# ParthaEth/GIF

Hardware: NVIDIA H100
Metric: G+D train step images/sec @256x256 bs32/GPU (higher is better)
Workload: dtype bf16x3 error-compensated tensor-core contraction (two-term bf16 operands, 3 MMAs per slice), f32 accumulate/storage

## Files before the change

gif_b200/_lib.py:

```python
import ctypes
import os

import torch

_HERE = os.path.dirname(os.path.abspath(__file__))
LIB_PATH = os.path.join(_HERE, "libgifb200.so")

_p = ctypes.c_void_p
_i = ctypes.c_int
_f = ctypes.c_float
_d = ctypes.c_double
_ll = ctypes.c_longlong
_sz = ctypes.c_size_t

SIGNATURES = {
    "gifb200_version": (_i, []),
    "gifb200_last_error": (ctypes.c_char_p, []),
    "gifb200_launch_count": (_ll, []),
    "gifb200_conv2d_workspace_bytes": (_sz, [_i] * 11),
    "gifb200_conv2d": (_i, [_p, _p, _p] + [_i] * 13 + [_p, _f, _f, _i, _p, _sz, _p]),
    "gifb200_conv2d_wgrad_workspace_bytes": (_sz, [_i] * 10),
    "gifb200_conv2d_wgrad_path": (_i, [_i] * 10),
    "gifb200_conv2d_wgrad": (_i, [_p, _p, _p] + [_i] * 12 + [_p, _sz, _p]),
    "gifb200_conv2d_ex_workspace_bytes": (_sz, [_i] * 13),
    "gifb200_conv2d_ex": (_i, [_p, _p, _p] + [_i] * 16 + [_p, _i, _p, _sz, _p]),
    "gifb200_pool2d": (_i, [_p, _p] + [_i] * 12 + [_p]),
    "gifb200_resize_bilinear": (_i, [_p, _p, _i, _i, _i, _ll, _ll, _ll, _ll, _i, _i, _i, _f, _f, _i, _p]),
    "gifb200_resize_bilinear_u8": (_i, [_p, _p, _i, _i, _i, _ll, _i, _i, _i, _f, _f, _i, _p]),
    "gifb200_split_bf16": (_i, [_p, _p, _p, _i, _i, _i, _p]),
    "gifb200_upfirdn2d": (_i, [_p, _p, _p] + [_i] * 14 + [_p]),
    "gifb200_bias_act": (_i, [_p, _p, _p, _p, _p, _i, _i, _i, _f, _f, _i, _p]),
    "gifb200_act_bwd": (_i, [_p, _p, _p, _ll, _f, _f, _i, _p]),
    "gifb200_rows_sum": (_i, [_p, _p, _i, _i, _i, _p]),
    "gifb200_chan_scale": (_i, [_p, _p, _p, _i, _i, _i, _i, _p]),
    "gifb200_tail_bwd": (_i, [_p] * 8 + [_i, _i, _i, _f, _f, _i, _p]),
# ... 86 lines not shown
```

gif_b200/csrc/conv_api.cu:

```cuda
#include "common.cuh"

namespace gifb200 {
int conv2d_simt(const float* x, const float* w, float* y, int B, int Hi, int Wi, int Ci, int Ho, int Wo, int Co, int k,
                int mode, int flip, int transposed, const ConvEpilogue& epi, cudaStream_t st);
int conv2d_wgrad_simt(const float* x, const float* gy, float* gw, int B, int Hi, int Wi, int Ci, int Ho, int Wo, int Co,
                      int k, int mode, int flip, int transposed, cudaStream_t st);
bool conv2d_tc_supported(int B, int Hi, int Wi, int Ci, int Ho, int Wo, int Co, int k, int mode);
size_t conv2d_tc_workspace_bytes(int B, int Hi, int Wi, int Ci, int Ho, int Wo, int Co, int k, int mode, int transposed);
int conv2d_tc(const float* x, const float* w, float* y, int B, int Hi, int Wi, int Ci, int Ho, int Wo, int Co, int k,
              int mode, int flip, int transposed, const ConvEpilogue& epi, void* ws, size_t ws_bytes, cudaStream_t st,
              bool x3, bool prestaged);
bool conv2d_wgrad_tc_supported(int B, int Hi, int Wi, int Ci, int Ho, int Wo, int Co, int k, int mode);
size_t conv2d_wgrad_tc_workspace_bytes(int B, int Hi, int Wi, int Ci, int Ho, int Wo, int Co, int k, int mode);
int conv2d_wgrad_tc(const float* x, const float* gy, float* gw, int B, int Hi, int Wi, int Ci, int Ho, int Wo, int Co,
                    int k, int mode, int flip, int transposed, void* ws, size_t ws_bytes, cudaStream_t st, bool x3);
}

using namespace gifb200;

extern "C" size_t gifb200_conv2d_workspace_bytes(int B, int Hi, int Wi, int Ci, int Ho, int Wo, int Co, int k, int mode,
                                                 int transposed, int impl) {
    impl &= 0xF;
    if (impl == 1) return 0;
    if (!conv2d_tc_supported(B, Hi, Wi, Ci, Ho, Wo, Co, k, mode)) return 0;
    return conv2d_tc_workspace_bytes(B, Hi, Wi, Ci, Ho, Wo, Co, k, mode, transposed);
}
// ... 4 lines not shown
                              gifb200_stream_t stream) {
    cudaStream_t st = static_cast<cudaStream_t>(stream);
    const ConvEpilogue epi{act, bias, slope, gain, round_tf32};
    const bool prestaged = (impl & GIFB200_CONV_PRESTAGED) != 0;
    impl &= 0xF;
    GIFB200_REQUIRE(impl >= 0 && impl <= 3, GIFB200_E_SHAPE,
                    "conv2d: impl must be 0 (auto), 1 (simt), 2 (wgmma tf32) or 3 (wgmma bf16x3 on split planes)");
    const bool tc_ok = conv2d_tc_supported(B, Hi, Wi, Ci, Ho, Wo, Co, k, mode);
    if (impl >= 2 && !tc_ok) return fail(GIFB200_E_SHAPE, "conv2d: shape not supported by the tensor-core path");
    if (impl != 1 && tc_ok)
        return conv2d_tc(x, w, y, B, Hi, Wi, Ci, Ho, Wo, Co, k, mode, flip, transposed, epi, workspace, workspace_bytes, st,
                         impl == 3, prestaged);
    return conv2d_simt(x, w, y, B, Hi, Wi, Ci, Ho, Wo, Co, k, mode, flip, transposed, epi, st);
}

extern "C" size_t gifb200_conv2d_wgrad_workspace_bytes(int B, int Hi, int Wi, int Ci, int Ho, int Wo, int Co, int k,
                                                       int mode, int impl) {
    if (impl == 1) return 0;
    return conv2d_wgrad_tc_workspace_bytes(B, Hi, Wi, Ci, Ho, Wo, Co, k, mode);
}

extern "C" int gifb200_conv2d_wgrad_path(int B, int Hi, int Wi, int Ci, int Ho, int Wo, int Co, int k, int mode, int impl) {
    if (impl == 1) return 1;
    if (conv2d_wgrad_tc_supported(B, Hi, Wi, Ci, Ho, Wo, Co, k, mode)) return impl == 3 ? 3 : 2;
    return impl == 0 ? 1 : 0;
}

extern "C" int gifb200_conv2d_wgrad(const float* x, const float* gy, float* gw, int B, int Hi, int Wi, int Ci, int Ho,
                                    int Wo, int Co, int k, int mode, int flip, int transposed, int impl, void* workspace,
                                    size_t workspace_bytes, gifb200_stream_t stream) {
// ... 10 lines not shown
```

gif_b200/csrc/conv_tc.cu:

```cuda
#include <cuda_bf16.h>

#include "tc_common.cuh"

namespace gifb200 {

namespace {

constexpr int kBlockK = 32;
constexpr int kMaxTaps = 9;
constexpr int kConsumerWarps = 8;

struct TcParams {
    int B, Hs, Ws;
    int wt, ht, nt;
    int tiles_x, tiles_y;
    int Ci, Co;
    int s2;
    int Ho, Wo;
    int oys, oxs;
    int nphase;
    int phase_oy0[4], phase_ox0[4], phase_ntaps[4];
    int tap_w[4][kMaxTaps];
    int tap_dy[4][kMaxTaps];
    int tap_dx[4][kMaxTaps];
    int tap_par[4][kMaxTaps];
    int in_sy;
    int ksplit;
    float* part;
    long long part_stride;
    ConvEpilogue epi;
};

constexpr int kProducerRegs = 40, kConsumerRegs = 232;
template <int BM, int BN>
struct TileCfg {
    static constexpr bool kLarge = BM * BN > 128 * 128;
    static constexpr int kRowBlocks = BM / 128;
    static constexpr int kAcc = kRowBlocks * BN / 2;
    static constexpr int kStages = kLarge ? 4 : 3;
    static constexpr int kThreads = kLarge ? 384 : 32 * kConsumerWarps + 32;
    static constexpr int kMinBlocks = kLarge ? 1 : 2;
    static constexpr int kATileBytes = BM * kBlockK * 4;
    static constexpr int kBTileBytes = BN * kBlockK * 4;
    static constexpr int kStageBytes = kATileBytes + kBTileBytes;
    static constexpr int kBarrierOffset = kStages * kStageBytes;
    static constexpr int kTotal = kBarrierOffset + 16 * kStages;
    static constexpr int kDynamic = kTotal + 1024;
    static_assert(kDynamic <= 227 * 1024, "shared memory ring too large");
};

__device__ __forceinline__ void decode_tile(int tile, int nblocks, int nphase, int rot_div, int& mt, int& nblk, int& phase) {
    const int inner = nblocks * nphase;
    mt = tile / inner;
    const int rem = tile - mt * inner;
    nblk = rem % nblocks;
    phase = nphase == 1 ? 0 : (rem / nblocks + mt / rot_div) % nphase;
}

template <int BM, int BN, bool X3>
__global__ void __launch_bounds__(TileCfg<BM, BN>::kThreads, TileCfg<BM, BN>::kMinBlocks)
    conv_tc_kernel(const __grid_constant__ CUtensorMap map_a, const __grid_constant__ CUtensorMap map_a2,
                   const __grid_constant__ CUtensorMap map_b, const __grid_constant__ CUtensorMap map_b2,
                   float* __restrict__ y, const TcParams p, const int mtiles, const int total_tiles) {
    using L = TileCfg<BM, BN>;
    constexpr int kStages = L::kStages;
    constexpr int kATileBytes = L::kATileBytes;
    extern __shared__ uint8_t smem_raw[];
    uint8_t* smem = reinterpret_cast<uint8_t*>((reinterpret_cast<uintptr_t>(smem_raw) + 1023) & ~static_cast<uintptr_t>(1023));
    uint64_t* full_bar = reinterpret_cast<uint64_t*>(smem + L::kBarrierOffset);
    uint64_t* empty_bar = full_bar + kStages;

    const int warp = threadIdx.x >> 5, lane = threadIdx.x & 31;
    const int nblocks = p.Co / BN;
    const int kchunks = p.Ci / kBlockK;
    const int rot_div = max(1, static_cast<int>(gridDim.x) / (nblocks * p.nphase));
    (void)mtiles;

    if (warp == kConsumerWarps && lane == 0) {
        asm volatile("prefetch.tensormap [%0];" ::"l"(&map_a) : "memory");
        asm volatile("prefetch.tensormap [%0];" ::"l"(&map_b) : "memory");
        if (X3) {
            asm volatile("prefetch.tensormap [%0];" ::"l"(&map_a2) : "memory");
            asm volatile("prefetch.tensormap [%0];" ::"l"(&map_b2) : "memory");
        }
        for (int s = 0; s < kStages; ++s) { mbar_init(&full_bar[s], 1); mbar_init(&empty_bar[s], 2); }
        asm volatile("fence.mbarrier_init.release.cluster;" ::: "memory");
        asm volatile("fence.proxy.async.shared::cta;" ::: "memory");
    }
    __syncthreads();

    if (warp >= kConsumerWarps) {
        if constexpr (L::kLarge) setmaxnreg_dec<kProducerRegs>();
        if (warp != kConsumerWarps) return;
        int stage = 0;
        uint32_t ph = 0;
        for (int tile = blockIdx.x; tile < total_tiles; tile += gridDim.x) {
            int mt, nblk, phase;
            const int ks = tile % p.ksplit;
            decode_tile(tile / p.ksplit, nblocks, p.nphase, rot_div, mt, nblk, phase);
            int m = mt;
            const int tx = m % p.tiles_x; m /= p.tiles_x;
            const int ty = m % p.tiles_y; m /= p.tiles_y;
            const int n0 = m * p.nt, y0 = ty * p.ht, x0 = tx * p.wt;
            const int iters = p.phase_ntaps[phase] * kchunks;
            const int it0 = iters * ks / p.ksplit, it1 = iters * (ks + 1) / p.ksplit;
            for (int it = it0; it < it1; ++it) {
                const int tap = it / kchunks, c0 = (it % kchunks) * kBlockK;
                uint8_t* a_dst = smem + stage * L::kStageBytes;
                uint8_t* b_dst = a_dst + kATileBytes;
                if (lane == 0) {
                    mbar_wait(&empty_bar[stage], ph ^ 1);
                    mbar_expect_tx(&full_bar[stage], L::kStageBytes);
                }
                __syncwarp();
                const int dy = p.tap_dy[phase][tap], dx = p.tap_dx[phase][tap];
                if (!p.s2) {
                    if (lane == 0) {
                        tma_load_4d(a_dst, &map_a, &full_bar[stage], c0, x0 + dx, y0 + dy, n0);
// ... 20 lines not shown
                }
                if (lane == 0) {
                    tma_load_3d(b_dst, &map_b, &full_bar[stage], c0, nblk * BN, p.tap_w[phase][tap]);
                    if (X3) tma_load_3d(b_dst + L::kBTileBytes / 2, &map_b2, &full_bar[stage], c0, nblk * BN, p.tap_w[phase][tap]);
                }
                if (++stage == kStages) { stage = 0; ph ^= 1; }
            }
        }
    } else {
        if constexpr (L::kLarge) setmaxnreg_inc<kConsumerRegs>();
        const int wg = warp >> 2;
        const int wq = warp & 3;
        constexpr int kRB = L::kRowBlocks;
        constexpr int kAcc = L::kAcc;
        float acc[kAcc];
        int w_in[2 * kRB], h_in[2 * kRB], n_in[2 * kRB];
#pragma unroll
        for (int rh = 0; rh < 2 * kRB; ++rh) {
            const int r = wg * (BM / 2) + (rh >> 1) * 64 + wq * 16 + (lane >> 2) + 8 * (rh & 1);
            w_in[rh] = r % p.wt; h_in[rh] = (r / p.wt) % p.ht; n_in[rh] = r / (p.wt * p.ht);
        }
        int stage = 0;
        uint32_t ph = 0;
        for (int tile = blockIdx.x; tile < total_tiles; tile += gridDim.x) {
            int mt, nblk, phase;
            const int ks = tile % p.ksplit;
            decode_tile(tile / p.ksplit, nblocks, p.nphase, rot_div, mt, nblk, phase);
            const int iters = p.phase_ntaps[phase] * kchunks;
            const int it0 = iters * ks / p.ksplit, it1 = iters * (ks + 1) / p.ksplit;
            int prev = -1;
            for (int it = it0; it < it1; ++it) {
                mbar_wait(&full_bar[stage], ph);
                const uint32_t a_addr = smem_u32(smem + stage * L::kStageBytes);
                wgmma_fence();
                fence_regs<kAcc>(acc);
                if (X3) {
                    const uint32_t a_wg = a_addr + wg * (BM / 2) * 64;
                    const uint64_t bh = make_kmajor_sw64_desc(a_addr + kATileBytes);
                    const uint64_t bl = make_kmajor_sw64_desc(a_addr + kATileBytes + L::kBTileBytes / 2);
#pragma unroll
                    for (int k = 0; k < kBlockK / 16; ++k) {
#pragma unroll
                        for (int rb = 0; rb < kRB; ++rb) {
                            const uint64_t ah = make_kmajor_sw64_desc(a_wg + rb * 64 * 64);
                            const uint64_t al = make_kmajor_sw64_desc(a_wg + rb * 64 * 64 + kATileBytes / 2);
                            float* d = acc + rb * (BN / 2);
                            wgmma_bf16<BN>(d, al + 2 * k, bh + 2 * k, (it != it0) || k != 0, Trans<0>());
                            wgmma_bf16<BN>(d, ah + 2 * k, bl + 2 * k, 1, Trans<0>());
                            wgmma_bf16<BN>(d, ah + 2 * k, bh + 2 * k, 1, Trans<0>());
                        }
                    }
                } else {
                    const uint64_t bdesc = make_kmajor_sw128_desc(a_addr + kATileBytes);
#pragma unroll
                    for (int k = 0; k < kBlockK / 8; ++k) {
#pragma unroll
                        for (int rb = 0; rb < kRB; ++rb) {
                            const uint64_t adesc = make_kmajor_sw128_desc(a_addr + (wg * (BM / 2) + rb * 64) * 128);
                            wgmma_tf32<BN>(acc + rb * (BN / 2), adesc + 2 * k, bdesc + 2 * k, (it != it0) || k != 0);
                        }
                    }
                }
                wgmma_commit();
                fence_regs<kAcc>(acc);
                wgmma_wait<1>();
                if (prev >= 0 && (threadIdx.x & 127) == 0) mbar_arrive(&empty_bar[prev]);
                prev = stage;
                if (++stage == kStages) { stage = 0; ph ^= 1; }
            }
            wgmma_wait<0>();
            fence_regs<kAcc>(acc);
            if (prev >= 0 && (threadIdx.x & 127) == 0) mbar_arrive(&empty_bar[prev]);
            int m = mt;
            const int tx = m % p.tiles_x; m /= p.tiles_x;
            const int ty = m % p.tiles_y; m /= p.tiles_y;
            float* base = p.ksplit > 1 ? p.part + ks * p.part_stride : y;
            const int c0 = nblk * BN + 2 * (lane & 3);
#pragma unroll
            for (int rh = 0; rh < 2 * kRB; ++rh) {
                const int h = rh & 1;
                const float* a = acc + (rh >> 1) * (BN / 2);
                const int n = m * p.nt + n_in[rh];
                const int Y = (ty * p.ht + h_in[rh]) * p.oys + p.phase_oy0[phase], X = (tx * p.wt + w_in[rh]) * p.oxs + p.phase_ox0[phase];
                if (n < p.B && Y < p.Ho && X < p.Wo) {
                    float* dst = base + ((static_cast<long long>(n) * p.Ho + Y) * p.Wo + X) * p.Co + c0;
#pragma unroll
                    for (int j = 0; j < BN / 8; ++j) {
                        float2 v = make_float2(a[4 * j + 2 * h], a[4 * j + 2 * h + 1]);
                        if (p.epi.act && p.ksplit == 1) {
                            v.x = apply_epilogue(p.epi, v.x, c0 + 8 * j);
                            v.y = apply_epilogue(p.epi, v.y, c0 + 8 * j + 1);
                        }
                        *reinterpret_cast<float2*>(dst + 8 * j) = v;
                    }
                }
            }
        }
    }
}

template <bool X3>
__global__ void __launch_bounds__(256) stage_weights_kernel(const float* __restrict__ w, float* __restrict__ out, int T,
                                                            int Co, int Ci, int flip, int transposed) {
    const long long total = static_cast<long long>(T) * Co * Ci;
    for (long long e = static_cast<long long>(blockIdx.x) * blockDim.x + threadIdx.x; e < total;
         e += static_cast<long long>(gridDim.x) * blockDim.x) {
        const int i = static_cast<int>(e % Ci);
        const int o = static_cast<int>((e / Ci) % Co);
        const int t = static_cast<int>(e / (static_cast<long long>(Ci) * Co));
        const int tt = flip ? T - 1 - t : t;
        const float v = transposed ? w[(static_cast<long long>(tt) * Ci + i) * Co + o]
                                   : w[(static_cast<long long>(tt) * Co + o) * Ci + i];
        if (X3) {
// ... 78 lines not shown
            a = fmaf(__bfloat162float(xv[i]) + __bfloat162float(xv[x_plane + i]),
                     __bfloat162float(wv[i]) + __bfloat162float(wv[w_plane + i]), a);
    } else {
        const float* xv = static_cast<const float*>(xpix_v) + b * x_batch_stride;
        const float* wv = static_cast<const float*>(w22_v) + static_cast<long long>(o) * Ci;
        for (int i = lane; i < Ci; i += 32) a = fmaf(xv[i], wv[i], a);
    }
    a = warp_sum(a);
    if (lane == 0) y[((static_cast<long long>(b) * Ho + (Ho - 1)) * Wo + (Wo - 1)) * Co + o] = apply_epilogue(epi, a, o);
}

void site_grid(int Hi, int Wi, int Ho, int Wo, int mode, int& Hs, int& Ws) {
    if (mode == 2) { Hs = Hi; Ws = Wi; } else { Hs = Ho; Ws = Wo; }
}

template <int BM, int BN, bool X3>
int launch(const CUtensorMap& ma, const CUtensorMap& ma2, const CUtensorMap& mb, const CUtensorMap& mb2, float* y,
           const TcParams& p, int mtiles, cudaStream_t st) {
    using L = TileCfg<BM, BN>;
    static bool attr_set = false;
    if (!attr_set) {
        cudaError_t e = cudaFuncSetAttribute(conv_tc_kernel<BM, BN, X3>, cudaFuncAttributeMaxDynamicSharedMemorySize, L::kDynamic);
        if (e != cudaSuccess) return fail(GIFB200_E_CUDA, "cudaFuncSetAttribute(conv_tc_kernel)", cudaGetErrorString(e));
        attr_set = true;
    }
    const long long total = static_cast<long long>(mtiles) * (p.Co / BN) * p.nphase * p.ksplit;
    if (total > 2147483647LL) return fail(GIFB200_E_SHAPE, "conv2d_tc: too many tiles");
    constexpr int kMaxGrid = L::kMinBlocks * kNumSMs;
    const int grid = total < kMaxGrid ? static_cast<int>(total) : kMaxGrid;
    conv_tc_kernel<BM, BN, X3><<<grid, L::kThreads, L::kDynamic, st>>>(ma, ma2, mb, mb2, y, p, mtiles, static_cast<int>(total));
    GIFB200_LAUNCH_CHECK("conv_tc_kernel");
    return GIFB200_OK;
}

template <bool X3>
int launch_tile(int bm, int bn, const CUtensorMap& ma, const CUtensorMap& ma2, const CUtensorMap& mb, const CUtensorMap& mb2,
                float* y, const TcParams& p, int mtiles, cudaStream_t st) {
    if (bm == 256) return launch<256, 128, X3>(ma, ma2, mb, mb2, y, p, mtiles, st);
    if (bn == 256) return launch<128, 256, X3>(ma, ma2, mb, mb2, y, p, mtiles, st);
    if (bn == 128) return launch<128, 128, X3>(ma, ma2, mb, mb2, y, p, mtiles, st);
    if (bn == 64) return launch<128, 64, X3>(ma, ma2, mb, mb2, y, p, mtiles, st);
    return launch<128, 32, X3>(ma, ma2, mb, mb2, y, p, mtiles, st);
}

int launch_any(int bm, int bn, bool x3, const CUtensorMap& ma, const CUtensorMap& ma2, const CUtensorMap& mb,
               const CUtensorMap& mb2, float* y, const TcParams& p, int mtiles, cudaStream_t st) {
    return x3 ? launch_tile<true>(bm, bn, ma, ma2, mb, mb2, y, p, mtiles, st)
              : launch_tile<false>(bm, bn, ma, ma2, mb, mb2, y, p, mtiles, st);
}

}

bool conv2d_tc_supported(int B, int Hi, int Wi, int Ci, int Ho, int Wo, int Co, int k, int mode) {
    if (B <= 0 || Ci % 32 != 0 || pick_block_n(Co) == 0) return false;
    if (!(k == 3 || (k == 1 && mode == 0))) return false;
    if (mode == 0 && !(Ho == Hi && Wo == Wi)) return false;
    if (mode == 1 && !(Hi == 2 * Ho + 1 && Wi == 2 * Wo + 1)) return false;
    if (mode == 2 && !(Ho == 2 * Hi + 1 && Wo == 2 * Wi + 1)) return false;
    int Hs, Ws;
    site_grid(Hi, Wi, Ho, Wo, mode, Hs, Ws);
    if (!pow2(Hs) || !pow2(Ws) || Ws < 4 || Hs < 4 || Ws > 4096 || Hs > 4096) return false;
    return true;
}

static size_t staged_weight_bytes(int Ci, int Co, int k) {
    return (static_cast<size_t>(k) * k * Co * Ci * sizeof(float) + 256 + 255) / 256 * 256;
}

static int ksplit_of(int B, int Hi, int Wi, int Ci, int Ho, int Wo, int Co, int k, int mode) {
    int Hs, Ws, wt, ht, nt;
    long long mtiles;
    site_grid(Hi, Wi, Ho, Wo, mode, Hs, Ws);
    tile_geometry(B, Hs, Ws, 128, wt, ht, nt, mtiles);
    const int bn = pick_block_n(Co);
    if (bn == 0) return 1;
    return pick_ksplit(mtiles * (Co / bn), k * k * (Ci / kBlockK), mode);
}

size_t conv2d_tc_workspace_bytes(int B, int Hi, int Wi, int Ci, int Ho, int Wo, int Co, int k, int mode, int) {
    size_t bytes = staged_weight_bytes(Ci, Co, k);
    if (conv2d_tc_supported(B, Hi, Wi, Ci, Ho, Wo, Co, k, mode)) {
        const int ks = ksplit_of(B, Hi, Wi, Ci, Ho, Wo, Co, k, mode);
        if (ks > 1) bytes += static_cast<size_t>(ks) * B * Ho * Wo * Co * sizeof(float) + 256;
    }
    return bytes;
}

int conv2d_tc(const float* x, const float* w, float* y, int B, int Hi, int Wi, int Ci, int Ho, int Wo, int Co, int k,
              int mode, int flip, int transposed, const ConvEpilogue& epi, void* ws, size_t ws_bytes, cudaStream_t st,
              bool x3, bool prestaged) {
    GIFB200_REQUIRE(conv2d_tc_supported(B, Hi, Wi, Ci, Ho, Wo, Co, k, mode), GIFB200_E_SHAPE, "conv2d_tc: unsupported shape");
// ... 23 lines not shown
    site_grid(Hi, Wi, Ho, Wo, mode, p.Hs, p.Ws);
    p.ksplit = ksplit_of(B, Hi, Wi, Ci, Ho, Wo, Co, k, mode);
    int bm, bn;
    pick_tile(B, p.Hs, p.Ws, Co, mode == 2 ? 4 : 1, p.ksplit, bm, bn);
    long long mtiles;
    tile_geometry(B, p.Hs, p.Ws, bm, p.wt, p.ht, p.nt, mtiles);
    p.tiles_x = p.Ws / p.wt; p.tiles_y = p.Hs / p.ht;
    GIFB200_REQUIRE(mtiles <= 2147483647LL, GIFB200_E_SHAPE, "conv2d_tc: too many tiles");
    if (p.ksplit > 1) {
        p.part_stride = static_cast<long long>(B) * Ho * Wo * Co;
        p.part = reinterpret_cast<float*>((reinterpret_cast<uintptr_t>(reinterpret_cast<char*>(wst) + staged_weight_bytes(Ci, Co, k) - 256) + 255) &
                                          ~static_cast<uintptr_t>(255));
    }
    p.s2 = mode == 1;
    p.in_sy = mode == 1 ? 2 : 1;
    const int pad = k / 2;
    if (mode == 0) {
        p.nphase = 1; p.oys = p.oxs = 1; p.phase_ntaps[0] = T;
        for (int t = 0; t < T; ++t) { p.tap_w[0][t] = t; p.tap_dy[0][t] = t / k - pad; p.tap_dx[0][t] = t % k - pad; }
    } else if (mode == 1) {
        p.nphase = 1; p.oys = p.oxs = 1; p.phase_ntaps[0] = T;
        for (int t = 0; t < T; ++t) {
            const int kh = t / k, kw = t % k;
            p.tap_w[0][t] = t; p.tap_dy[0][t] = kh; p.tap_dx[0][t] = kw >> 1; p.tap_par[0][t] = kw & 1;
        }
    } else {
        p.nphase = 4; p.oys = p.oxs = 2;
        for (int ph = 0; ph < 4; ++ph) {
            const int py = ph >> 1, px = ph & 1;
            p.phase_oy0[ph] = py; p.phase_ox0[ph] = px;
            int n = 0;
            for (int kh = py; kh < 3; kh += 2)
                for (int kw = px; kw < 3; kw += 2) {
                    p.tap_w[ph][n] = kh * 3 + kw; p.tap_dy[ph][n] = (py - kh) / 2; p.tap_dx[ph][n] = (px - kw) / 2;
                    ++n;
                }
            p.phase_ntaps[ph] = n;
        }
    }
    CUtensorMap ma, ma2, mb, mb2;
    int rc;
    if (mode != 1) {
        const cuuint64_t dims[4] = {static_cast<cuuint64_t>(Ci), static_cast<cuuint64_t>(Wi), static_cast<cuuint64_t>(Hi), static_cast<cuuint64_t>(B)};
        const cuuint64_t strides[3] = {static_cast<cuuint64_t>(Ci) * es, static_cast<cuuint64_t>(Wi) * Ci * es,
                                       static_cast<cuuint64_t>(Hi) * Wi * Ci * es};
        const cuuint32_t box[4] = {kBlockK, static_cast<cuuint32_t>(p.wt), static_cast<cuuint32_t>(p.ht), static_cast<cuuint32_t>(p.nt)};
        rc = encode_map(&ma, xb, 4, dims, strides, box, swz, dt);
        if (rc == GIFB200_OK && x3) rc = encode_map(&ma2, xb + x_plane * es, 4, dims, strides, box, swz, dt);
    } else {
        const cuuint64_t dims[5] = {static_cast<cuuint64_t>(Ci), 2, static_cast<cuuint64_t>((Wi + 1) / 2), static_cast<cuuint64_t>(Hi), static_cast<cuuint64_t>(B)};
        const cuuint64_t strides[4] = {static_cast<cuuint64_t>(Ci) * es, static_cast<cuuint64_t>(Ci) * 2 * es,
                                       static_cast<cuuint64_t>(Wi) * Ci * es, static_cast<cuuint64_t>(Hi) * Wi * Ci * es};
        static const bool per_row = [] { const char* e = getenv("GIFB200_CONV_S2_ROWS"); return e && atoi(e) != 0; }();
        const bool onebox = !per_row && p.ht * p.nt > 1;
        if (onebox) p.s2 = 2;
        const cuuint32_t box[5] = {kBlockK, 1, static_cast<cuuint32_t>(p.wt), static_cast<cuuint32_t>(onebox ? 2 * p.ht : 1),
                                   static_cast<cuuint32_t>(onebox ? p.nt : 1)};
        const cuuint32_t estr[5] = {1, 1, 1, static_cast<cuuint32_t>(onebox ? 2 : 1), 1};
        rc = encode_map(&ma, xb, 5, dims, strides, box, swz, dt, estr);
        if (rc == GIFB200_OK && x3) rc = encode_map(&ma2, xb + x_plane * es, 5, dims, strides, box, swz, dt, estr);
    }
    if (rc != GIFB200_OK) return rc;
    auto encode_b = [&](int box_n, CUtensorMap& m, CUtensorMap& m2) {
        const cuuint64_t dims[3] = {static_cast<cuuint64_t>(Ci), static_cast<cuuint64_t>(Co), static_cast<cuuint64_t>(T)};
        const cuuint64_t strides[2] = {static_cast<cuuint64_t>(Ci) * es, static_cast<cuuint64_t>(Co) * Ci * es};
        const cuuint32_t box[3] = {kBlockK, static_cast<cuuint32_t>(box_n), 1};
        int r = encode_map(&m, wb, 3, dims, strides, box, swz, dt);
        if (r == GIFB200_OK && x3) r = encode_map(&m2, wb + w_plane * es, 3, dims, strides, box, swz, dt);
        if (!x3) m2 = m;
        return r;
    };
    rc = encode_b(bn, mb, mb2);
    if (rc != GIFB200_OK) return rc;
    if (!x3) ma2 = ma;
    rc = launch_any(bm, bn, x3, ma, ma2, mb, mb2, y, p, static_cast<int>(mtiles), st);
    if (rc == GIFB200_OK && p.ksplit > 1) {
        const long long n4 = p.part_stride / 4;
        int blocks = cdiv(n4, 256);
        if (blocks > kNumSMs * 8) blocks = kNumSMs * 8;
        splitk_reduce_kernel<<<blocks, 256, 0, st>>>(p.part, y, n4, p.ksplit, p.part_stride, epi, Co);
        GIFB200_LAUNCH_CHECK("splitk_reduce_kernel");
    }
    if (mode != 2 || rc != GIFB200_OK) return rc;
    const int bn_e = pick_block_n(Co);
    CUtensorMap mbe = mb, mbe2 = mb2;
    if (bn_e != bn) rc = encode_b(bn_e, mbe, mbe2);
    for (int edge = 0; edge < 2 && rc == GIFB200_OK; ++edge) {
        const bool row = edge == 0;
        TcParams q;
        memset(&q, 0, sizeof(q));
// ... 16 lines not shown
                ++n;
            }
            q.phase_ntaps[ph] = n;
        }
        CUtensorMap me, me2;
        const char* base = xb + (row ? static_cast<long long>(Hi - 1) * Wi * Ci : static_cast<long long>(Wi - 1) * Ci) * es;
        const cuuint64_t dims[4] = {static_cast<cuuint64_t>(Ci), static_cast<cuuint64_t>(row ? Wi : 1),
                                    static_cast<cuuint64_t>(row ? 1 : Hi), static_cast<cuuint64_t>(B)};
        const cuuint64_t strides[3] = {static_cast<cuuint64_t>(Ci) * es, static_cast<cuuint64_t>(Wi) * Ci * es,
                                       static_cast<cuuint64_t>(Hi) * Wi * Ci * es};
        const cuuint32_t box[4] = {kBlockK, static_cast<cuuint32_t>(q.wt), static_cast<cuuint32_t>(q.ht), static_cast<cuuint32_t>(q.nt)};
        rc = encode_map(&me, base, 4, dims, strides, box, swz, dt);
        if (rc == GIFB200_OK && x3) rc = encode_map(&me2, base + x_plane * es, 4, dims, strides, box, swz, dt);
        if (rc != GIFB200_OK) return rc;
        if (!x3) me2 = me;
        rc = launch_any(128, bn_e, x3, me, me2, mbe, mbe2, y, q, static_cast<int>(mt_e), st);
    }
    if (rc != GIFB200_OK) return rc;
    {
        const char* xpix = xb + (static_cast<long long>(Hi - 1) * Wi + (Wi - 1)) * Ci * es;
        const char* w22 = wb + static_cast<long long>(8) * Co * Ci * es;
        const int blocks = cdiv(static_cast<long long>(B) * Co * 32, 256);
        if (x3)
            t2_corner_kernel<true><<<blocks, 256, 0, st>>>(xpix, w22, y, B, static_cast<long long>(Hi) * Wi * Ci, Ci, Co, Ho, Wo,
                                                           epi, x_plane, w_plane);
        else
            t2_corner_kernel<false><<<blocks, 256, 0, st>>>(xpix, w22, y, B, static_cast<long long>(Hi) * Wi * Ci, Ci, Co, Ho, Wo,
                                                            epi, 0, 0);
    }
    GIFB200_LAUNCH_CHECK("t2_corner_kernel");
    return rc;
// ... 4 lines not shown
```

include/gifb200.h:

```cpp
#ifndef GIFB200_H
#define GIFB200_H

#include <stddef.h>
#include <stdint.h>

#ifdef __cplusplus
extern "C" {
#endif

#define GIFB200_OK 0
#define GIFB200_E_SHAPE (-1)
#define GIFB200_E_ALIGN (-2)
#define GIFB200_E_ARCH (-3)
#define GIFB200_E_CUDA (-4)
#define GIFB200_E_WORKSPACE (-5)

typedef void* gifb200_stream_t;

int gifb200_version(void);
const char* gifb200_last_error(void);
long long gifb200_launch_count(void);

#define GIFB200_CONV_PRESTAGED 0x10
size_t gifb200_conv2d_workspace_bytes(int B, int Hi, int Wi, int Ci, int Ho, int Wo, int Co, int k, int mode,
                                      int transposed, int impl);
int gifb200_conv2d(const float* x, const float* w, float* y, int B, int Hi, int Wi, int Ci, int Ho, int Wo, int Co,
                   int k, int mode, int flip, int transposed, int impl, int act, const float* bias, float slope,
                   float gain, int round_tf32, void* workspace, size_t workspace_bytes, gifb200_stream_t stream);

size_t gifb200_conv2d_wgrad_workspace_bytes(int B, int Hi, int Wi, int Ci, int Ho, int Wo, int Co, int k, int mode,
                                            int impl);
int gifb200_conv2d_wgrad_path(int B, int Hi, int Wi, int Ci, int Ho, int Wo, int Co, int k, int mode, int impl);
int gifb200_conv2d_wgrad(const float* x, const float* gy, float* gw, int B, int Hi, int Wi, int Ci, int Ho, int Wo,
                         int Co, int k, int mode, int flip, int transposed, int impl, void* workspace,
                         size_t workspace_bytes, gifb200_stream_t stream);

size_t gifb200_conv2d_ex_workspace_bytes(int B, int Hi, int Wi, int Ci, int Ho, int Wo, int Co, int kh, int kw, int stride,
                                         int pad_h, int pad_w, int impl);
int gifb200_conv2d_ex(const void* x, const float* w, float* y, int B, int Hi, int Wi, int Ci, int Ho, int Wo, int Co, int kh,
                      int kw, int stride, int pad_h, int pad_w, int Cy, int c0, int impl, int act, const float* bias,
                      int round_tf32, void* workspace, size_t workspace_bytes, gifb200_stream_t stream);
int gifb200_pool2d(const float* x, float* y, int B, int Hi, int Wi, int C, int Ho, int Wo, int stride, int pad, int op, int Cy,
                   int c0, int round_tf32, gifb200_stream_t stream);
// ... 116 lines not shown
```

Before: 82.39.

## Add halo-tile A loading for 3x3 stride-1 tensor-core convolutions

Adds a halo variant of the TMA/wgmma implicit-GEMM conv kernel for 3x3 stride-1 forward convolutions. Instead of issuing one A-tile load per tap, each input row band is loaded once with a two-pixel halo and reused across the three horizontal taps by offsetting the shared-memory descriptor. A and B get separate barrier rings. This removes redundant global/L2 traffic for A, at the cost of a more complex pipeline and a shared-memory layout that can reduce the number of B stages. The path is on by default and can be disabled with an environment variable; a path-query API is also exposed.

After: 82.28 (median of 6 runs). Within noise of the previous version (-0.1%).

```diff
diff --git a/gif_b200/_lib.py b/gif_b200/_lib.py
--- a/gif_b200/_lib.py
+++ b/gif_b200/_lib.py
@@ -19,6 +19,7 @@
     "gifb200_launch_count": (_ll, []),
     "gifb200_conv2d_workspace_bytes": (_sz, [_i] * 11),
     "gifb200_conv2d": (_i, [_p, _p, _p] + [_i] * 13 + [_p, _f, _f, _i, _p, _sz, _p]),
+    "gifb200_conv2d_path": (_i, [_i] * 10),
     "gifb200_conv2d_wgrad_workspace_bytes": (_sz, [_i] * 10),
     "gifb200_conv2d_wgrad_path": (_i, [_i] * 10),
     "gifb200_conv2d_wgrad": (_i, [_p, _p, _p] + [_i] * 12 + [_p, _sz, _p]),
diff --git a/gif_b200/csrc/conv_api.cu b/gif_b200/csrc/conv_api.cu
--- a/gif_b200/csrc/conv_api.cu
+++ b/gif_b200/csrc/conv_api.cu
@@ -10,6 +10,7 @@
 int conv2d_tc(const float* x, const float* w, float* y, int B, int Hi, int Wi, int Ci, int Ho, int Wo, int Co, int k,
               int mode, int flip, int transposed, const ConvEpilogue& epi, void* ws, size_t ws_bytes, cudaStream_t st,
               bool x3, bool prestaged);
+int conv2d_tc_path(int B, int Hi, int Wi, int Ci, int Ho, int Wo, int Co, int k, int mode, bool x3);
 bool conv2d_wgrad_tc_supported(int B, int Hi, int Wi, int Ci, int Ho, int Wo, int Co, int k, int mode);
 size_t conv2d_wgrad_tc_workspace_bytes(int B, int Hi, int Wi, int Ci, int Ho, int Wo, int Co, int k, int mode);
 int conv2d_wgrad_tc(const float* x, const float* gy, float* gw, int B, int Hi, int Wi, int Ci, int Ho, int Wo, int Co,
@@ -44,6 +45,13 @@
     return conv2d_simt(x, w, y, B, Hi, Wi, Ci, Ho, Wo, Co, k, mode, flip, transposed, epi, st);
 }
 
+extern "C" int gifb200_conv2d_path(int B, int Hi, int Wi, int Ci, int Ho, int Wo, int Co, int k, int mode, int impl) {
+    impl &= 0xF;
+    if (impl == 1) return 1;
+    if (conv2d_tc_supported(B, Hi, Wi, Ci, Ho, Wo, Co, k, mode)) return conv2d_tc_path(B, Hi, Wi, Ci, Ho, Wo, Co, k, mode, impl == 3);
+    return impl == 0 ? 1 : 0;
+}
+
 extern "C" size_t gifb200_conv2d_wgrad_workspace_bytes(int B, int Hi, int Wi, int Ci, int Ho, int Wo, int Co, int k,
                                                        int mode, int impl) {
     if (impl == 1) return 0;
diff --git a/gif_b200/csrc/conv_tc.cu b/gif_b200/csrc/conv_tc.cu
--- a/gif_b200/csrc/conv_tc.cu
+++ b/gif_b200/csrc/conv_tc.cu
@@ -25,6 +25,10 @@
     int tap_dx[4][kMaxTaps];
     int tap_par[4][kMaxTaps];
     int in_sy;
+    int halo_line;
+    int halo_slot;
+    int halo_bslots;
+    int halo_off[2][2];
     int ksplit;
     float* part;
     long long part_stride;
@@ -32,7 +36,9 @@
 };
 
 constexpr int kProducerRegs = 40, kConsumerRegs = 232;
-template <int BM, int BN>
+constexpr int kHaloMaxA = 8, kHaloMaxB = 8;
+constexpr int kHaloAOffset = 1024;
+template <int BM, int BN, bool HALO = false>
 struct TileCfg {
     static constexpr bool kLarge = BM * BN > 128 * 128;
     static constexpr int kRowBlocks = BM / 128;
@@ -43,10 +49,11 @@
     static constexpr int kATileBytes = BM * kBlockK * 4;
     static constexpr int kBTileBytes = BN * kBlockK * 4;
     static constexpr int kStageBytes = kATileBytes + kBTileBytes;
-    static constexpr int kBarrierOffset = kStages * kStageBytes;
-    static constexpr int kTotal = kBarrierOffset + 16 * kStages;
-    static constexpr int kDynamic = kTotal + 1024;
+    static constexpr int kBarriers = HALO ? kHaloMaxA + kHaloMaxB : kStages;
+    static constexpr int kBarrierOffset = HALO ? 0 : kStages * kStageBytes;
+    static constexpr int kDynamic = HALO ? (kLarge ? 227 * 1024 : 112 * 1024) : kStages * kStageBytes + 16 * kStages + 1024;
     static_assert(kDynamic <= 227 * 1024, "shared memory ring too large");
+    static_assert(kLarge || 2 * (kDynamic + 1024) <= 228 * 1024, "128 x BN tiles must keep two CTAs per SM");
 };
 
 __device__ __forceinline__ void decode_tile(int tile, int nblocks, int nphase, int rot_div, int& mt, int& nblk, int& phase) {
@@ -57,22 +64,25 @@
     phase = nphase == 1 ? 0 : (rem / nblocks + mt / rot_div) % nphase;
 }
 
-template <int BM, int BN, bool X3>
-__global__ void __launch_bounds__(TileCfg<BM, BN>::kThreads, TileCfg<BM, BN>::kMinBlocks)
-    conv_tc_kernel(const __grid_constant__ CUtensorMap map_a, const __grid_constant__ CUtensorMap map_a2,
-                   const __grid_constant__ CUtensorMap map_b, const __grid_constant__ CUtensorMap map_b2,
-                   float* __restrict__ y, const TcParams p, const int mtiles, const int total_tiles) {
-    using L = TileCfg<BM, BN>;
+template <int BM, int BN, bool X3, bool HALO>
+__device__ __forceinline__ void conv_tc_body(const CUtensorMap& map_a, const CUtensorMap& map_a2, const CUtensorMap& map_b,
+                                             const CUtensorMap& map_b2, float* __restrict__ y, const TcParams& p,
+                                             const int mtiles, const int total_tiles) {
+    using L = TileCfg<BM, BN, HALO>;
     constexpr int kStages = L::kStages;
     constexpr int kATileBytes = L::kATileBytes;
     extern __shared__ uint8_t smem_raw[];
     uint8_t* smem = reinterpret_cast<uint8_t*>((reinterpret_cast<uintptr_t>(smem_raw) + 1023) & ~static_cast<uintptr_t>(1023));
     uint64_t* full_bar = reinterpret_cast<uint64_t*>(smem + L::kBarrierOffset);
-    uint64_t* empty_bar = full_bar + kStages;
+    uint64_t* empty_bar = full_bar + L::kBarriers;
+    uint64_t* full_b = full_bar + kHaloMaxA;
+    uint64_t* empty_b = empty_bar + kHaloMaxA;
+    constexpr int kRowBytes = X3 ? 64 : 128;
 
     const int warp = threadIdx.x >> 5, lane = threadIdx.x & 31;
     const int nblocks = p.Co / BN;
     const int kchunks = p.Ci / kBlockK;
+    const int aslots = kchunks < 2 ? 2 : kchunks;
     const int rot_div = max(1, static_cast<int>(gridDim.x) / (nblocks * p.nphase));
     (void)mtiles;
 
@@ -83,7 +93,7 @@
             asm volatile("prefetch.tensormap [%0];" ::"l"(&map_a2) : "memory");
             asm volatile("prefetch.tensormap [%0];" ::"l"(&map_b2) : "memory");
         }
-        for (int s = 0; s < kStages; ++s) { mbar_init(&full_bar[s], 1); mbar_init(&empty_bar[s], 2); }
+        for (int s = 0; s < L::kBarriers; ++s) { mbar_init(&full_bar[s], 1); mbar_init(&empty_bar[s], 2); }
         asm volatile("fence.mbarrier_init.release.cluster;" ::: "memory");
         asm volatile("fence.proxy.async.shared::cta;" ::: "memory");
     }
@@ -102,6 +112,43 @@
             const int tx = m % p.tiles_x; m /= p.tiles_x;
             const int ty = m % p.tiles_y; m /= p.tiles_y;
             const int n0 = m * p.nt, y0 = ty * p.ht, x0 = tx * p.wt;
+            if constexpr (HALO) {
+                const int lines = p.nt * p.ht;
+                const uint32_t a_tx = lines * (p.wt + 2) * 128;
+                const int ln_n = lane / p.ht, ln_y = y0 + lane - ln_n * p.ht - 1;
+                const uint32_t tl = (tile - blockIdx.x) / gridDim.x;
+                for (int it = 0; it < 9 * kchunks; ++it) {
+                    const int tap = it / kchunks, c = it - tap * kchunks, kh = tap / 3;
+                    if (tap == 3 * kh) {
+                        const uint32_t box = (3 * tl + kh) * kchunks + c;
+                        const int as = box % aslots;
+                        uint8_t* a_dst = smem + kHaloAOffset + as * p.halo_slot + lane * p.halo_line;
+                        if (lane == 0) {
+                            mbar_wait(&empty_bar[as], ((box / aslots) & 1) ^ 1);
+                            mbar_expect_tx(&full_bar[as], a_tx);
+                        }
+                        __syncwarp();
+                        if (lane < lines) {
+                            tma_load_4d(a_dst, &map_a, &full_bar[as], c * kBlockK, x0 - 1, ln_y + kh, n0 + ln_n);
+                            if (X3)
+                                tma_load_4d(a_dst + lines * p.halo_line, &map_a2, &full_bar[as], c * kBlockK, x0 - 1, ln_y + kh,
+                                            n0 + ln_n);
+                        }
+                    }
+                    if (lane == 0) {
+                        const uint32_t bi = 9 * kchunks * tl + it;
+                        const int bs = bi % p.halo_bslots;
+                        uint8_t* b_dst = smem + kHaloAOffset + aslots * p.halo_slot + bs * L::kBTileBytes;
+                        mbar_wait(&empty_b[bs], ((bi / p.halo_bslots) & 1) ^ 1);
+                        mbar_expect_tx(&full_b[bs], L::kBTileBytes);
+                        const int tw = p.tap_w[0][tap];
+                        tma_load_3d(b_dst, &map_b, &full_b[bs], c * kBlockK, nblk * BN, tw);
+                        if (X3) tma_load_3d(b_dst + L::kBTileBytes / 2, &map_b2, &full_b[bs], c * kBlockK, nblk * BN, tw);
+                    }
+                    __syncwarp();
+                }
+                continue;
+            }
             const int iters = p.phase_ntaps[phase] * kchunks;
             const int it0 = iters * ks / p.ksplit, it1 = iters * (ks + 1) / p.ksplit;
             for (int it = it0; it < it1; ++it) {
@@ -152,11 +199,14 @@
         constexpr int kRB = L::kRowBlocks;
         constexpr int kAcc = L::kAcc;
         float acc[kAcc];
-        int w_in[2 * kRB], h_in[2 * kRB], n_in[2 * kRB];
-#pragma unroll
-        for (int rh = 0; rh < 2 * kRB; ++rh) {
+        auto site_of = [&](int rh) -> uint32_t {
             const int r = wg * (BM / 2) + (rh >> 1) * 64 + wq * 16 + (lane >> 2) + 8 * (rh & 1);
-            w_in[rh] = r % p.wt; h_in[rh] = (r / p.wt) % p.ht; n_in[rh] = r / (p.wt * p.ht);
+            return (r % p.wt) | ((r / p.wt) % p.ht) << 8 | (r / (p.wt * p.ht)) << 16;
+        };
+        uint32_t site_in[2 * kRB];
+        if constexpr (!HALO) {
+#pragma unroll
+            for (int rh = 0; rh < 2 * kRB; ++rh) site_in[rh] = site_of(rh);
         }
         int stage = 0;
         uint32_t ph = 0;
@@ -167,48 +217,106 @@
             const int iters = p.phase_ntaps[phase] * kchunks;
             const int it0 = iters * ks / p.ksplit, it1 = iters * (ks + 1) / p.ksplit;
             int prev = -1;
-            for (int it = it0; it < it1; ++it) {
-                mbar_wait(&full_bar[stage], ph);
-                const uint32_t a_addr = smem_u32(smem + stage * L::kStageBytes);
-                wgmma_fence();
+            if constexpr (HALO) {
+                const uint32_t tl = (tile - blockIdx.x) / gridDim.x;
+                for (int it = 0; it < iters; ++it) {
+                    const int tap = it / kchunks, c = it - tap * kchunks, kh = tap / 3, kw = tap - 3 * kh;
+                    const uint32_t box = (3 * tl + kh) * kchunks + c;
+                    const int as = box % aslots;
+                    if (kw == 0) mbar_wait(&full_bar[as], (box / aslots) & 1);
+                    const uint32_t bi = iters * tl + it;
+                    const int bs = bi % p.halo_bslots;
+                    mbar_wait(&full_b[bs], (bi / p.halo_bslots) & 1);
+                    const uint32_t a_addr = smem_u32(smem + kHaloAOffset + as * p.halo_slot) + kw * kRowBytes;
+                    const uint32_t b_addr = smem_u32(smem + kHaloAOffset + aslots * p.halo_slot + bs * L::kBTileBytes);
+                    wgmma_fence();
+                    fence_regs<kAcc>(acc);
+                    if (X3) {
+                        const uint32_t a_lo = p.nt * p.ht * p.halo_line;
+                        const uint64_t bh = make_kmajor_sw64_desc(b_addr);
+                        const uint64_t bl = make_kmajor_sw64_desc(b_addr + L::kBTileBytes / 2);
+#pragma unroll
+                        for (int k = 0; k < kBlockK / 16; ++k) {
+#pragma unroll
+                            for (int rb = 0; rb < kRB; ++rb) {
+                                const uint64_t ah = make_kmajor_sw64_desc(a_addr + p.halo_off[wg][rb]);
+                                const uint64_t al = make_kmajor_sw64_desc(a_addr + p.halo_off[wg][rb] + a_lo);
+                                float* d = acc + rb * (BN / 2);
+                                wgmma_bf16<BN>(d, al + 2 * k, bh + 2 * k, it != 0 || k != 0, Trans<0>());
+                                wgmma_bf16<BN>(d, ah + 2 * k, bl + 2 * k, 1, Trans<0>());
+                                wgmma_bf16<BN>(d, ah + 2 * k, bh + 2 * k, 1, Trans<0>());
+                            }
+                        }
+                    } else {
+                        const uint64_t bdesc = make_kmajor_sw128_desc(b_addr);
+#pragma unroll
+                        for (int k = 0; k < kBlockK / 8; ++k) {
+#pragma unroll
+                            for (int rb = 0; rb < kRB; ++rb) {
+                                const uint64_t adesc = make_kmajor_sw128_desc(a_addr + p.halo_off[wg][rb]);
+                                wgmma_tf32<BN>(acc + rb * (BN / 2), adesc + 2 * k, bdesc + 2 * k, it != 0 || k != 0);
+                            }
+                        }
+                    }
+                    wgmma_commit();
+                    fence_regs<kAcc>(acc);
+                    wgmma_wait<1>();
+                    if ((threadIdx.x & 127) == 0 && it != 0) {
+                        mbar_arrive(&empty_b[(bi - 1) % p.halo_bslots]);
+                        const int ptap = (it - 1) / kchunks;
+                        if (ptap % 3 == 2) mbar_arrive(&empty_bar[((3 * tl + ptap / 3) * kchunks + (it - 1) - ptap * kchunks) % aslots]);
+                    }
+                }
+                wgmma_wait<0>();
                 fence_regs<kAcc>(acc);
-                if (X3) {
-                    const uint32_t a_wg = a_addr + wg * (BM / 2) * 64;
-                    const uint64_t bh = make_kmajor_sw64_desc(a_addr + kATileBytes);
-                    const uint64_t bl = make_kmajor_sw64_desc(a_addr + kATileBytes + L::kBTileBytes / 2);
-#pragma unroll
-                    for (int k = 0; k < kBlockK / 16; ++k) {
-#pragma unroll
-                        for (int rb = 0; rb < kRB; ++rb) {
-                            const uint64_t ah = make_kmajor_sw64_desc(a_wg + rb * 64 * 64);
-                            const uint64_t al = make_kmajor_sw64_desc(a_wg + rb * 64 * 64 + kATileBytes / 2);
-                            float* d = acc + rb * (BN / 2);
-                            wgmma_bf16<BN>(d, al + 2 * k, bh + 2 * k, (it != it0) || k != 0, Trans<0>());
-                            wgmma_bf16<BN>(d, ah + 2 * k, bl + 2 * k, 1, Trans<0>());
-                            wgmma_bf16<BN>(d, ah + 2 * k, bh + 2 * k, 1, Trans<0>());
+                if ((threadIdx.x & 127) == 0) {
+                    mbar_arrive(&empty_b[(iters * tl + iters - 1) % p.halo_bslots]);
+                    mbar_arrive(&empty_bar[((3 * tl + 3) * kchunks - 1) % aslots]);
+                }
+            } else {
+                for (int it = it0; it < it1; ++it) {
+                    mbar_wait(&full_bar[stage], ph);
+                    const uint32_t a_addr = smem_u32(smem + stage * L::kStageBytes);
+                    wgmma_fence();
+                    fence_regs<kAcc>(acc);
+                    if (X3) {
+                        const uint32_t a_wg = a_addr + wg * (BM / 2) * 64;
+                        const uint64_t bh = make_kmajor_sw64_desc(a_addr + kATileBytes);
+                        const uint64_t bl = make_kmajor_sw64_desc(a_addr + kATileBytes + L::kBTileBytes / 2);
+#pragma unroll
+                        for (int k = 0; k < kBlockK / 16; ++k) {
+#pragma unroll
+                            for (int rb = 0; rb < kRB; ++rb) {
+                                const uint64_t ah = make_kmajor_sw64_desc(a_wg + rb * 64 * 64);
+                                const uint64_t al = make_kmajor_sw64_desc(a_wg + rb * 64 * 64 + kATileBytes / 2);
+                                float* d = acc + rb * (BN / 2);
+                                wgmma_bf16<BN>(d, al + 2 * k, bh + 2 * k, (it != it0) || k != 0, Trans<0>());
+                                wgmma_bf16<BN>(d, ah + 2 * k, bl + 2 * k, 1, Trans<0>());
+                                wgmma_bf16<BN>(d, ah + 2 * k, bh + 2 * k, 1, Trans<0>());
+                            }
                         }
-                    }
-                } else {
-                    const uint64_t bdesc = make_kmajor_sw128_desc(a_addr + kATileBytes);
-#pragma unroll
-                    for (int k = 0; k < kBlockK / 8; ++k) {
-#pragma unroll
-                        for (int rb = 0; rb < kRB; ++rb) {
-                            const uint64_t adesc = make_kmajor_sw128_desc(a_addr + (wg * (BM / 2) + rb * 64) * 128);
-                            wgmma_tf32<BN>(acc + rb * (BN / 2), adesc + 2 * k, bdesc + 2 * k, (it != it0) || k != 0);
+                    } else {
+                        const uint64_t bdesc = make_kmajor_sw128_desc(a_addr + kATileBytes);
+#pragma unroll
+                        for (int k = 0; k < kBlockK / 8; ++k) {
+#pragma unroll
+                            for (int rb = 0; rb < kRB; ++rb) {
+                                const uint64_t adesc = make_kmajor_sw128_desc(a_addr + (wg * (BM / 2) + rb * 64) * 128);
+                                wgmma_tf32<BN>(acc + rb * (BN / 2), adesc + 2 * k, bdesc + 2 * k, (it != it0) || k != 0);
+                            }
                         }
                     }
-                }
-                wgmma_commit();
+                    wgmma_commit();
+                    fence_regs<kAcc>(acc);
+                    wgmma_wait<1>();
+                    if (prev >= 0 && (threadIdx.x & 127) == 0) mbar_arrive(&empty_bar[prev]);
+                    prev = stage;
+                    if (++stage == kStages) { stage = 0; ph ^= 1; }
+                }
+                wgmma_wait<0>();
                 fence_regs<kAcc>(acc);
-                wgmma_wait<1>();
                 if (prev >= 0 && (threadIdx.x & 127) == 0) mbar_arrive(&empty_bar[prev]);
-                prev = stage;
-                if (++stage == kStages) { stage = 0; ph ^= 1; }
             }
-            wgmma_wait<0>();
-            fence_regs<kAcc>(acc);
-            if (prev >= 0 && (threadIdx.x & 127) == 0) mbar_arrive(&empty_bar[prev]);
             int m = mt;
             const int tx = m % p.tiles_x; m /= p.tiles_x;
             const int ty = m % p.tiles_y; m /= p.tiles_y;
@@ -218,8 +326,10 @@
             for (int rh = 0; rh < 2 * kRB; ++rh) {
                 const int h = rh & 1;
                 const float* a = acc + (rh >> 1) * (BN / 2);
-                const int n = m * p.nt + n_in[rh];
-                const int Y = (ty * p.ht + h_in[rh]) * p.oys + p.phase_oy0[phase], X = (tx * p.wt + w_in[rh]) * p.oxs + p.phase_ox0[phase];
+                const uint32_t site = HALO ? site_of(rh) : site_in[rh];
+                const int w_in = site & 255, h_in = (site >> 8) & 255, n_in = site >> 16;
+                const int n = m * p.nt + n_in;
+                const int Y = (ty * p.ht + h_in) * p.oys + p.phase_oy0[phase], X = (tx * p.wt + w_in) * p.oxs + p.phase_ox0[phase];
                 if (n < p.B && Y < p.Ho && X < p.Wo) {
                     float* dst = base + ((static_cast<long long>(n) * p.Ho + Y) * p.Wo + X) * p.Co + c0;
 #pragma unroll
@@ -235,6 +345,21 @@
             }
         }
     }
+}
+
+template <int BM, int BN, bool X3>
+__global__ void __launch_bounds__(TileCfg<BM, BN>::kThreads, TileCfg<BM, BN>::kMinBlocks)
+    conv_tc_kernel(const __grid_constant__ CUtensorMap map_a, const __grid_constant__ CUtensorMap map_a2,
+                   const __grid_constant__ CUtensorMap map_b, const __grid_constant__ CUtensorMap map_b2,
+                   float* __restrict__ y, const TcParams p, const int mtiles, const int total_tiles) {
+    conv_tc_body<BM, BN, X3, false>(map_a, map_a2, map_b, map_b2, y, p, mtiles, total_tiles);
+}
+template <int BM, int BN, bool X3>
+__global__ void __launch_bounds__(TileCfg<BM, BN>::kThreads, TileCfg<BM, BN>::kMinBlocks)
+    conv_tc_kernel_halo(const __grid_constant__ CUtensorMap map_a, const __grid_constant__ CUtensorMap map_a2,
+                        const __grid_constant__ CUtensorMap map_b, const __grid_constant__ CUtensorMap map_b2,
+                        float* __restrict__ y, const TcParams p, const int mtiles, const int total_tiles) {
+    conv_tc_body<BM, BN, X3, true>(map_a, map_a2, map_b, map_b2, y, p, mtiles, total_tiles);
 }
 
 template <bool X3>
@@ -343,13 +468,14 @@
     if (mode == 2) { Hs = Hi; Ws = Wi; } else { Hs = Ho; Ws = Wo; }
 }
 
-template <int BM, int BN, bool X3>
+template <int BM, int BN, bool X3, bool HALO>
 int launch(const CUtensorMap& ma, const CUtensorMap& ma2, const CUtensorMap& mb, const CUtensorMap& mb2, float* y,
            const TcParams& p, int mtiles, cudaStream_t st) {
-    using L = TileCfg<BM, BN>;
+    using L = TileCfg<BM, BN, HALO>;
+    const auto kernel = HALO ? conv_tc_kernel_halo<BM, BN, X3> : conv_tc_kernel<BM, BN, X3>;
     static bool attr_set = false;
     if (!attr_set) {
-        cudaError_t e = cudaFuncSetAttribute(conv_tc_kernel<BM, BN, X3>, cudaFuncAttributeMaxDynamicSharedMemorySize, L::kDynamic);
+        cudaError_t e = cudaFuncSetAttribute(kernel, cudaFuncAttributeMaxDynamicSharedMemorySize, L::kDynamic);
         if (e != cudaSuccess) return fail(GIFB200_E_CUDA, "cudaFuncSetAttribute(conv_tc_kernel)", cudaGetErrorString(e));
         attr_set = true;
     }
@@ -357,25 +483,33 @@
     if (total > 2147483647LL) return fail(GIFB200_E_SHAPE, "conv2d_tc: too many tiles");
     constexpr int kMaxGrid = L::kMinBlocks * kNumSMs;
     const int grid = total < kMaxGrid ? static_cast<int>(total) : kMaxGrid;
-    conv_tc_kernel<BM, BN, X3><<<grid, L::kThreads, L::kDynamic, st>>>(ma, ma2, mb, mb2, y, p, mtiles, static_cast<int>(total));
+    kernel<<<grid, L::kThreads, L::kDynamic, st>>>(ma, ma2, mb, mb2, y, p, mtiles, static_cast<int>(total));
     GIFB200_LAUNCH_CHECK("conv_tc_kernel");
     return GIFB200_OK;
 }
 
-template <bool X3>
+template <bool X3, bool HALO>
 int launch_tile(int bm, int bn, const CUtensorMap& ma, const CUtensorMap& ma2, const CUtensorMap& mb, const CUtensorMap& mb2,
                 float* y, const TcParams& p, int mtiles, cudaStream_t st) {
-    if (bm == 256) return launch<256, 128, X3>(ma, ma2, mb, mb2, y, p, mtiles, st);
-    if (bn == 256) return launch<128, 256, X3>(ma, ma2, mb, mb2, y, p, mtiles, st);
-    if (bn == 128) return launch<128, 128, X3>(ma, ma2, mb, mb2, y, p, mtiles, st);
-    if (bn == 64) return launch<128, 64, X3>(ma, ma2, mb, mb2, y, p, mtiles, st);
-    return launch<128, 32, X3>(ma, ma2, mb, mb2, y, p, mtiles, st);
-}
-
-int launch_any(int bm, int bn, bool x3, const CUtensorMap& ma, const CUtensorMap& ma2, const CUtensorMap& mb,
+    if (bm == 256) return launch<256, 128, X3, HALO>(ma, ma2, mb, mb2, y, p, mtiles, st);
+    if (bn == 256) return launch<128, 256, X3, HALO>(ma, ma2, mb, mb2, y, p, mtiles, st);
+    if (bn == 128) return launch<128, 128, X3, HALO>(ma, ma2, mb, mb2, y, p, mtiles, st);
+    if (bn == 64) return launch<128, 64, X3, HALO>(ma, ma2, mb, mb2, y, p, mtiles, st);
+    return launch<128, 32, X3, HALO>(ma, ma2, mb, mb2, y, p, mtiles, st);
+}
+
+int launch_any(int bm, int bn, bool x3, bool halo, const CUtensorMap& ma, const CUtensorMap& ma2, const CUtensorMap& mb,
                const CUtensorMap& mb2, float* y, const TcParams& p, int mtiles, cudaStream_t st) {
-    return x3 ? launch_tile<true>(bm, bn, ma, ma2, mb, mb2, y, p, mtiles, st)
-              : launch_tile<false>(bm, bn, ma, ma2, mb, mb2, y, p, mtiles, st);
+    if (halo)
+        return x3 ? launch_tile<true, true>(bm, bn, ma, ma2, mb, mb2, y, p, mtiles, st)
+                  : launch_tile<false, true>(bm, bn, ma, ma2, mb, mb2, y, p, mtiles, st);
+    return x3 ? launch_tile<true, false>(bm, bn, ma, ma2, mb, mb2, y, p, mtiles, st)
+              : launch_tile<false, false>(bm, bn, ma, ma2, mb, mb2, y, p, mtiles, st);
+}
+
+bool halo_enabled() {
+    static const bool on = [] { const char* e = getenv("GIFB200_CONV_HALO"); return !e || atoi(e) != 0; }();
+    return on;
 }
 
 }
@@ -404,6 +538,35 @@
     const int bn = pick_block_n(Co);
     if (bn == 0) return 1;
     return pick_ksplit(mtiles * (Co / bn), k * k * (Ci / kBlockK), mode);
+}
+
+static bool halo_layout(int bm, int bn, bool x3, int wt, int Ci, int& line, int& slot, int& bslots) {
+    const int row_bytes = x3 ? 64 : 128;
+    const int aslots = Ci / kBlockK < 2 ? 2 : Ci / kBlockK;
+    line = ((wt + 2) * row_bytes + 1023) & ~1023;
+    slot = (bm / wt) * line * (x3 ? 2 : 1);
+    const bool large = bm * bn > 128 * 128;
+    const int budget = (large ? TileCfg<256, 128, true>::kDynamic : TileCfg<128, 128, true>::kDynamic) - 1024 -
+                       kHaloAOffset;
+    bslots = (budget - aslots * slot) / (bn * kBlockK * 4);
+    if (bslots > 6) bslots = 6;
+    return aslots <= kHaloMaxA && bslots >= 3;
+}
+
+static bool halo_path(int mode, int k, int ksplit, int bm, int bn, bool x3, int wt, int Ci) {
+    int line, slot, bslots;
+    return halo_enabled() && mode == 0 && k == 3 && ksplit == 1 && wt % 64 == 0 &&
+           halo_layout(bm, bn, x3, wt, Ci, line, slot, bslots);
+}
+
+int conv2d_tc_path(int B, int Hi, int Wi, int Ci, int Ho, int Wo, int Co, int k, int mode, bool x3) {
+    int Hs, Ws, bm, bn, wt, ht, nt;
+    long long mtiles;
+    site_grid(Hi, Wi, Ho, Wo, mode, Hs, Ws);
+    const int ks = ksplit_of(B, Hi, Wi, Ci, Ho, Wo, Co, k, mode);
+    pick_tile(B, Hs, Ws, Co, mode == 2 ? 4 : 1, ks, bm, bn);
+    tile_geometry(B, Hs, Ws, bm, wt, ht, nt, mtiles);
+    return halo_path(mode, k, ks, bm, bn, x3, wt, Ci) ? 3 : 2;
 }
 
 size_t conv2d_tc_workspace_bytes(int B, int Hi, int Wi, int Ci, int Ho, int Wo, int Co, int k, int mode, int) {
@@ -457,6 +620,16 @@
     }
     p.s2 = mode == 1;
     p.in_sy = mode == 1 ? 2 : 1;
+    const bool halo = halo_path(mode, k, p.ksplit, bm, bn, x3, p.wt, Ci);
+    if (halo) {
+        const int row_bytes = x3 ? 64 : 128;
+        halo_layout(bm, bn, x3, p.wt, Ci, p.halo_line, p.halo_slot, p.halo_bslots);
+        for (int wg = 0; wg < 2; ++wg)
+            for (int rb = 0; rb < bm / 128; ++rb) {
+                const int r0 = wg * (bm / 2) + rb * 64;
+                p.halo_off[wg][rb] = (r0 / p.wt) * p.halo_line + (r0 % p.wt) * row_bytes;
+            }
+    }
     const int pad = k / 2;
     if (mode == 0) {
         p.nphase = 1; p.oys = p.oxs = 1; p.phase_ntaps[0] = T;
@@ -487,7 +660,8 @@
         const cuuint64_t dims[4] = {static_cast<cuuint64_t>(Ci), static_cast<cuuint64_t>(Wi), static_cast<cuuint64_t>(Hi), static_cast<cuuint64_t>(B)};
         const cuuint64_t strides[3] = {static_cast<cuuint64_t>(Ci) * es, static_cast<cuuint64_t>(Wi) * Ci * es,
                                        static_cast<cuuint64_t>(Hi) * Wi * Ci * es};
-        const cuuint32_t box[4] = {kBlockK, static_cast<cuuint32_t>(p.wt), static_cast<cuuint32_t>(p.ht), static_cast<cuuint32_t>(p.nt)};
+        const cuuint32_t box[4] = {kBlockK, static_cast<cuuint32_t>(halo ? p.wt + 2 : p.wt), static_cast<cuuint32_t>(halo ? 1 : p.ht),
+                                   static_cast<cuuint32_t>(halo ? 1 : p.nt)};
         rc = encode_map(&ma, xb, 4, dims, strides, box, swz, dt);
         if (rc == GIFB200_OK && x3) rc = encode_map(&ma2, xb + x_plane * es, 4, dims, strides, box, swz, dt);
     } else {
@@ -516,7 +690,7 @@
     rc = encode_b(bn, mb, mb2);
     if (rc != GIFB200_OK) return rc;
     if (!x3) ma2 = ma;
-    rc = launch_any(bm, bn, x3, ma, ma2, mb, mb2, y, p, static_cast<int>(mtiles), st);
+    rc = launch_any(bm, bn, x3, halo, ma, ma2, mb, mb2, y, p, static_cast<int>(mtiles), st);
     if (rc == GIFB200_OK && p.ksplit > 1) {
         const long long n4 = p.part_stride / 4;
         int blocks = cdiv(n4, 256);
@@ -563,7 +737,7 @@
         if (rc == GIFB200_OK && x3) rc = encode_map(&me2, base + x_plane * es, 4, dims, strides, box, swz, dt);
         if (rc != GIFB200_OK) return rc;
         if (!x3) me2 = me;
-        rc = launch_any(128, bn_e, x3, me, me2, mbe, mbe2, y, q, static_cast<int>(mt_e), st);
+        rc = launch_any(128, bn_e, x3, false, me, me2, mbe, mbe2, y, q, static_cast<int>(mt_e), st);
     }
     if (rc != GIFB200_OK) return rc;
     {
diff --git a/include/gifb200.h b/include/gifb200.h
--- a/include/gifb200.h
+++ b/include/gifb200.h
@@ -27,6 +27,7 @@
 int gifb200_conv2d(const float* x, const float* w, float* y, int B, int Hi, int Wi, int Ci, int Ho, int Wo, int Co,
                    int k, int mode, int flip, int transposed, int impl, int act, const float* bias, float slope,
                    float gain, int round_tf32, void* workspace, size_t workspace_bytes, gifb200_stream_t stream);
+int gifb200_conv2d_path(int B, int Hi, int Wi, int Ci, int Ho, int Wo, int Co, int k, int mode, int impl);
 
 size_t gifb200_conv2d_wgrad_workspace_bytes(int B, int Hi, int Wi, int Ci, int Ho, int Wo, int Co, int k, int mode,
                                             int impl);
```
